# Thealexbarney/VGAudio

Hardware: NVIDIA H100
Metric: GC-ADPCM encode Msamples/sec (batch) (higher is better)
Workload: dtype int32

## Files before the change

include/vgaudio_b200.h:

```cpp
#ifndef VGAUDIO_B200_H
#define VGAUDIO_B200_H

#include <stdint.h>

#ifdef __cplusplus
extern "C" {
#endif

#define VGB_OK        0
#define VGB_E_ARG    -1
#define VGB_E_DATA   -2
#define VGB_E_STATE  -3
#define VGB_E_CUDA   -4
#define VGB_E_NCCL   -5
#define VGB_E_NOMEM  -6

#define VGB_ABI_VERSION 1

int32_t vgb_abi_version(void);
int32_t vgb_init(int32_t device, uint32_t flags);
int32_t vgb_shutdown(void);
int32_t vgb_init_devices(const int32_t *devices, int32_t n_devices, uint32_t flags);
int32_t vgb_device_count(void);

// ... 52 lines not shown
                               void *d_workspace, uint64_t workspace_bytes, void *cuda_stream);

int32_t vgb_gcadpcm_coefs_dev(const int16_t *d_pcm, const int64_t *pcm_offset, const int32_t *n_samples,
                              int32_t n_channels, int16_t *d_coefs_out,
                              void *d_workspace, uint64_t workspace_bytes, void *cuda_stream);

int32_t vgb_gcadpcm_decode_dev(const uint8_t *d_adpcm, const int64_t *adpcm_offset, const int16_t *d_coefs,
                               const vgb_gc_params *params , int32_t n_channels,
                               int16_t *d_pcm, const int64_t *pcm_offset,
                               void *d_workspace, uint64_t workspace_bytes, void *cuda_stream);
int32_t vgb_gcadpcm_decode_dev_status(const void *d_workspace, int32_t n_channels, void *cuda_stream);

typedef struct vgb_gc_tap_params {
    int32_t sample_count;
    int32_t samples_per_seek_table_entry;
    int32_t loop_start;
} vgb_gc_tap_params;

int32_t vgb_gcadpcm_seek_entry_count(int32_t sample_count, int32_t samples_per_entry);

int32_t vgb_gcadpcm_seek_context_batch(const uint8_t *const *adpcm, const int32_t *n_bytes, const int16_t *coefs,
                                       const vgb_gc_tap_params *params, int32_t n_channels,
                                       int16_t *const *seek_table_out, int16_t *loop_context_out);

typedef struct vgb_gc_align_params { int32_t multiple, loop_start, loop_end; } vgb_gc_align_params;
typedef struct vgb_gc_alignment { int32_t alignment_needed, loop_start_aligned, sample_count_aligned; } vgb_gc_alignment;

int32_t vgb_gcadpcm_alignment(const vgb_gc_align_params *p, vgb_gc_alignment *out);

int32_t vgb_gcadpcm_align_batch(const uint8_t *const *adpcm, const int32_t *n_bytes, const int16_t *coefs,
                                const vgb_gc_align_params *params, int32_t n_channels,
                                uint8_t *const *adpcm_aligned_out, int16_t *const *pcm_aligned_out);

int32_t vgb_interleave_dev(const void *d_in, int64_t in_channel_stride, int64_t in_item_stride, void *d_out, int64_t out_item_stride,
                           int32_t n_items, int32_t count, int64_t in_size, int32_t interleave_size, int64_t out_size, void *cuda_stream);
int32_t vgb_deinterleave_dev(const void *d_in, int64_t in_item_stride, void *d_out, int64_t out_channel_stride, int64_t out_item_stride,
                             int32_t n_items, int32_t count, int64_t in_size, int32_t interleave_size, int64_t out_size, void *cuda_stream);
int32_t vgb_interleave(const uint8_t *const *inputs, int32_t count, int32_t in_size, int32_t interleave_size, int32_t out_size,
                       uint8_t *output);
int32_t vgb_deinterleave(const uint8_t *input, int32_t length, int32_t interleave_size, int32_t count, int32_t out_size,
                         uint8_t *const *outputs);

int32_t vgb_set_kernel_timing(int32_t enabled);
int32_t vgb_last_kernel_ms(float *ms_out, int32_t n);

int32_t vgb_debug_last_timeline(float *ms_out, int32_t n);
int32_t vgb_debug_last_coefs_done(float *ms_out, int32_t n);

int32_t vgb_gcadpcm_debug_splice_stats(uint64_t *out, int32_t n);

int32_t vgb_gcadpcm_debug_records(const int16_t *pcm, int32_t n_samples, double *dir_out, uint8_t *accepted_out);
int32_t vgb_gcadpcm_debug_refine_trace(const int16_t *const *pcm, const int32_t *n_samples, int32_t n_channels, int32_t warps,
                                       double *cent_out, int32_t *hits_out, int16_t *coefs_out);


typedef struct vgb_adx_params {
    int32_t sample_rate;
    int32_t highpass_frequency;
    int32_t frame_size;
    int32_t version;
    int32_t history;
    int32_t padding;
    int32_t type;
    int32_t filter;
} vgb_adx_params;

int32_t vgb_adx_calculate_coefficients(int32_t highpass_frequency, int32_t sample_rate, int16_t *coefs_out);

int32_t vgb_adx_encoded_byte_count(int32_t pcm_length, int32_t padding, int32_t frame_size);

int32_t vgb_adx_encode_batch(const int16_t *const *pcm, const int32_t *n_samples, const vgb_adx_params *params,
                             int32_t n_channels, int16_t *history_out, uint8_t *const *adpcm_out,
                             vgb_progress_cb cb, void *user);

uint64_t vgb_adx_workspace_bytes(int64_t total_samples, int32_t n_channels);
int32_t vgb_adx_encode_dev(const int16_t *d_pcm, const int64_t *pcm_offset, const int32_t *n_samples, const vgb_adx_params *params,
                           int32_t n_channels, int16_t *d_history_out, uint8_t *d_adpcm, const int64_t *adpcm_offset,
                           void *d_workspace, uint64_t workspace_bytes, void *cuda_stream);

int32_t vgb_adx_decode_batch(const uint8_t *const *adpcm, const int32_t *n_bytes, const int32_t *sample_count,
                             const vgb_adx_params *params, int32_t n_channels, int16_t *const *pcm_out);

uint64_t vgb_adx_decode_workspace_bytes(const int32_t *sample_count, const vgb_adx_params *params, int32_t n_channels);
int32_t vgb_adx_decode_dev(const uint8_t *d_adpcm, const int64_t *adpcm_offset, const int32_t *n_bytes, const int32_t *sample_count,
                           const vgb_adx_params *params, int32_t n_channels, int16_t *d_pcm, const int64_t *pcm_offset,
                           void *d_workspace, uint64_t workspace_bytes, void *cuda_stream);
int32_t vgb_adx_decode_dev_status(const void *d_workspace, int32_t n_channels, void *cuda_stream);
int32_t vgb_adx_debug_decode_stats(uint64_t *out, int32_t n);


typedef struct vgb_hca_params {
    int32_t quality, bitrate, limit_bitrate;
    int32_t channel_count, sample_rate, sample_count;
    int32_t looping, loop_start, loop_end;
} vgb_hca_params;

typedef struct vgb_hca_info {
    int32_t channel_count, sample_rate, sample_count, frame_count, inserted_samples, appended_samples;
    int32_t header_size, frame_size, min_resolution, max_resolution, track_count, channel_config;
    int32_t total_band_count, base_band_count, stereo_band_count, hfr_band_count, bands_per_hfr_group, hfr_group_count;
    int32_t bitrate;
    int32_t looping, loop_start_frame, loop_end_frame, pre_loop_samples, post_loop_samples;
    int32_t use_ath_curve;
} vgb_hca_info;

int32_t vgb_hca_query(const vgb_hca_params *params, vgb_hca_info *info_out);
// ... 119 lines not shown
```

vgaudio_b200/_native.py:

```python
from __future__ import annotations

import ctypes as C
import os

_HERE = os.path.dirname(os.path.abspath(__file__))
LIB_PATH = os.path.join(_HERE, "libvgaudio_b200.so")

VGB_OK, VGB_E_ARG, VGB_E_DATA, VGB_E_STATE, VGB_E_CUDA, VGB_E_NCCL, VGB_E_NOMEM = 0, -1, -2, -3, -4, -5, -6


class VgbGcParams(C.Structure):

    _fields_ = [("sample_count", C.c_int32), ("history1", C.c_int16), ("history2", C.c_int16)]


class VgbAdxParams(C.Structure):

    _fields_ = [("sample_rate", C.c_int32), ("highpass_frequency", C.c_int32), ("frame_size", C.c_int32),
                ("version", C.c_int32), ("history", C.c_int32), ("padding", C.c_int32), ("type", C.c_int32),
                ("filter", C.c_int32)]


class VgbHcaParams(C.Structure):

# ... 125 lines not shown
    "vgb_gcadpcm_coefs_dev": (
        C.c_int32,
        [C.c_void_p, C.c_void_p, C.c_void_p, C.c_int32, C.c_void_p, C.c_void_p, C.c_uint64, C.c_void_p],
    ),
    "vgb_gcadpcm_decode_dev": (
        C.c_int32,
        [C.c_void_p, C.c_void_p, C.c_void_p, C.c_void_p, C.c_int32, C.c_void_p, C.c_void_p, C.c_void_p, C.c_uint64,
         C.c_void_p],
    ),
    "vgb_gcadpcm_decode_dev_status": (C.c_int32, [C.c_void_p, C.c_int32, C.c_void_p]),
    "vgb_adx_encoded_byte_count": (C.c_int32, [C.c_int32, C.c_int32, C.c_int32]),
    "vgb_adx_encode_batch": (C.c_int32, [C.c_void_p, C.c_void_p, C.c_void_p, C.c_int32, C.c_void_p, C.c_void_p,
                                         C.c_void_p, C.c_void_p]),
    "vgb_adx_calculate_coefficients": (C.c_int32, [C.c_int32, C.c_int32, C.c_void_p]),
    "vgb_adx_decode_batch": (C.c_int32, [C.c_void_p, C.c_void_p, C.c_void_p, C.c_void_p, C.c_int32, C.c_void_p]),
    "vgb_adx_decode_workspace_bytes": (C.c_uint64, [C.c_void_p, C.c_void_p, C.c_int32]),
    "vgb_adx_decode_dev": (C.c_int32, [C.c_void_p, C.c_void_p, C.c_void_p, C.c_void_p, C.c_void_p, C.c_int32, C.c_void_p, C.c_void_p,
                                       C.c_void_p, C.c_uint64, C.c_void_p]),
    "vgb_adx_decode_dev_status": (C.c_int32, [C.c_void_p, C.c_int32, C.c_void_p]),
    "vgb_adx_debug_decode_stats": (C.c_int32, [C.c_void_p, C.c_int32]),
    "vgb_adx_workspace_bytes": (C.c_uint64, [C.c_int64, C.c_int32]),
    "vgb_adx_encode_dev": (C.c_int32, [C.c_void_p, C.c_void_p, C.c_void_p, C.c_void_p, C.c_int32, C.c_void_p, C.c_void_p, C.c_void_p,
                                       C.c_void_p, C.c_uint64, C.c_void_p]),
    "vgb_hca_workspace_bytes": (C.c_uint64, [C.c_int32]),
    "vgb_hca_encode_dev": (C.c_int32, [C.c_void_p, C.c_void_p, C.c_void_p, C.c_void_p, C.c_int32, C.c_void_p, C.c_void_p, C.c_void_p,
                                       C.c_void_p, C.c_uint64, C.c_void_p]),
    "vgb_hca_encode_dev_status": (C.c_int32, [C.c_void_p, C.c_int32, C.c_void_p]),
    "vgb_mdct128_batch": (C.c_int32, [C.c_void_p, C.c_int32, C.c_int32, C.c_void_p]),
    "vgb_imdct128_batch": (C.c_int32, [C.c_void_p, C.c_int32, C.c_int32, C.c_void_p]),
    "vgb_hca_query": (C.c_int32, [C.c_void_p, C.c_void_p]),
    "vgb_hca_encode_batch": (C.c_int32, [C.c_void_p, C.c_void_p, C.c_int32, C.c_void_p, C.c_void_p, C.c_void_p, C.c_void_p]),
    "vgb_hca_decode_batch": (C.c_int32, [C.c_void_p, C.c_void_p, C.c_int32, C.c_void_p]),
    "vgb_hca_decode_workspace_bytes": (C.c_uint64, [C.c_void_p, C.c_int32]),
    "vgb_hca_decode_dev": (C.c_int32, [C.c_void_p, C.c_void_p, C.c_void_p, C.c_int32, C.c_void_p, C.c_void_p, C.c_void_p, C.c_void_p,
                                       C.c_uint64, C.c_void_p]),
    "vgb_hca_decode_dev_status": (C.c_int32, [C.c_void_p, C.c_int32, C.c_void_p]),
    "vgb_gcadpcm_seek_entry_count": (C.c_int32, [C.c_int32, C.c_int32]),
    "vgb_gcadpcm_seek_context_batch": (C.c_int32, [C.c_void_p, C.c_void_p, C.c_void_p, C.c_void_p, C.c_int32, C.c_void_p, C.c_void_p]),
    "vgb_gcadpcm_alignment": (C.c_int32, [C.c_void_p, C.c_void_p]),
    "vgb_gcadpcm_align_batch": (C.c_int32, [C.c_void_p, C.c_void_p, C.c_void_p, C.c_void_p, C.c_int32, C.c_void_p, C.c_void_p]),
    "vgb_interleave_dev": (C.c_int32, [C.c_void_p, C.c_int64, C.c_int64, C.c_void_p, C.c_int64, C.c_int32, C.c_int32, C.c_int64,
                                       C.c_int32, C.c_int64, C.c_void_p]),
    "vgb_deinterleave_dev": (C.c_int32, [C.c_void_p, C.c_int64, C.c_void_p, C.c_int64, C.c_int64, C.c_int32, C.c_int32, C.c_int64,
                                         C.c_int32, C.c_int64, C.c_void_p]),
    "vgb_interleave": (C.c_int32, [C.c_void_p, C.c_int32, C.c_int32, C.c_int32, C.c_int32, C.c_void_p]),
    "vgb_deinterleave": (C.c_int32, [C.c_void_p, C.c_int32, C.c_int32, C.c_int32, C.c_int32, C.c_void_p]),
    "vgb_set_kernel_timing": (C.c_int32, [C.c_int32]),
    "vgb_last_kernel_ms": (C.c_int32, [C.c_void_p, C.c_int32]),
    "vgb_debug_last_timeline": (C.c_int32, [C.c_void_p, C.c_int32]),
    "vgb_debug_last_coefs_done": (C.c_int32, [C.c_void_p, C.c_int32]),
    "vgb_gcadpcm_debug_records": (C.c_int32, [C.c_void_p, C.c_int32, C.c_void_p, C.c_void_p]),
    "vgb_gcadpcm_debug_refine_trace": (C.c_int32, [C.c_void_p, C.c_void_p, C.c_int32, C.c_int32, C.c_void_p, C.c_void_p,
                                                   C.c_void_p]),
    "vgb_gcadpcm_debug_splice_stats": (C.c_int32, [C.c_void_p, C.c_int32]),
    "vgb_wave_parse": (C.c_int32, [C.c_void_p, C.c_int64, C.c_void_p]),
    "vgb_wave_read_batch": (C.c_int32, [C.c_void_p, C.c_void_p, C.c_void_p, C.c_int32, C.c_void_p]),
    "vgb_dsp_file_size": (C.c_int64, [C.c_void_p]),
    "vgb_dsp_write_batch": (C.c_int32, [C.c_void_p, C.c_int32, C.c_void_p, C.c_void_p, C.c_void_p, C.c_void_p, C.c_void_p, C.c_void_p]),
    "vgb_dsp_parse": (C.c_int32, [C.c_void_p, C.c_int64, C.c_void_p]),
    "vgb_dsp_read_batch": (C.c_int32, [C.c_void_p, C.c_void_p, C.c_void_p, C.c_int32, C.c_void_p]),
    "vgb_adx_key_from_code": (C.c_int32, [C.c_uint64, C.c_void_p]),
    "vgb_adx_key_from_string": (C.c_int32, [C.c_char_p, C.c_void_p]),
    "vgb_adx_file_size": (C.c_int64, [C.c_void_p]),
    "vgb_adx_write_batch": (C.c_int32, [C.c_void_p, C.c_int32, C.c_void_p, C.c_void_p, C.c_void_p, C.c_void_p, C.c_void_p]),
    "vgb_adx_crypt_batch": (C.c_int32, [C.c_void_p, C.c_int32, C.c_int32, C.c_void_p, C.c_int32, C.c_int32]),
    "vgb_adx_parse": (C.c_int32, [C.c_void_p, C.c_int64, C.c_void_p]),
    "vgb_hca_parse": (C.c_int32, [C.c_void_p, C.c_int64, C.c_void_p, C.c_void_p]),
    "vgb_hca_key_tables": (C.c_int32, [C.c_int32, C.c_uint64, C.c_void_p, C.c_void_p]),
    "vgb_hca_crypt_batch": (C.c_int32, [C.c_void_p, C.c_void_p, C.c_int32, C.c_int32, C.c_int32, C.c_uint64, C.c_int32]),
    "vgb_hca_write_batch": (C.c_int32, [C.c_void_p, C.c_int32, C.c_void_p, C.c_int32, C.c_uint64, C.c_void_p, C.c_void_p, C.c_void_p]),
    "vgb_convert_debug_stage_ms": (C.c_int32, [C.c_void_p, C.c_int32]),
    "vgb_convert_dsp_to_wave_batch": (C.c_int32, [C.c_void_p, C.c_void_p, C.c_int32, C.c_void_p, C.c_void_p, C.c_void_p]),
    "vgb_convert_hca_to_wave_batch": (C.c_int32, [C.c_void_p, C.c_void_p, C.c_int32, C.c_void_p, C.c_void_p, C.c_void_p, C.c_void_p]),
    "vgb_convert_adx_to_wave_batch": (C.c_int32, [C.c_void_p, C.c_void_p, C.c_int32, C.c_void_p, C.c_void_p, C.c_void_p, C.c_void_p]),
    "vgb_convert_wave_batch": (C.c_int32, [C.c_void_p, C.c_void_p, C.c_int32, C.c_void_p, C.c_void_p, C.c_void_p, C.c_void_p,
                                           C.c_void_p, C.c_void_p]),
    "vgb_transcode_batch": (C.c_int32, [C.c_void_p, C.c_void_p, C.c_void_p, C.c_int32, C.c_void_p, C.c_void_p, C.c_void_p,
                                        C.c_void_p, C.c_void_p, C.c_void_p, C.c_void_p, C.c_void_p]),
}


class VgbError(RuntimeError):

    def __init__(self, code: int, message: str):
        super().__init__(f"vgaudio_b200 error {code}: {message}")
        self.code = code


def _load() -> C.CDLL:
    if not os.path.exists(LIB_PATH):
        raise ImportError(
            f"{LIB_PATH} is missing: build it with `python -c 'import __graft_entry__ as g; g.build()'` "
            "(nvcc, sm_90a).  vgaudio_b200 has no CPU fallback."
        )
    lib = C.CDLL(LIB_PATH)
    for name, (res, args) in SIGNATURES.items():
        fn = getattr(lib, name)
        fn.restype = res
        fn.argtypes = args
    return lib


lib = _load()


def check(status: int) -> None:
# ... 3 lines not shown
```

vgaudio_b200/csrc/abi_gcadpcm.cu:

```cuda
#include <climits>

#include "abi.cuh"

using namespace vgb;

namespace {

struct GcLayout {
    int32_t n_channels = 0;
    std::vector<int64_t> pcm_off, adpcm_off, rec_off;
    std::vector<int32_t> n_samples, enc_count;
    std::vector<int16_t> hist;
    int64_t pcm_total = 0;
    int64_t adpcm_total = 0;
    int64_t rec_total = 0;
    int32_t max_frames = 0;
    int64_t total_frames = 0;
};

struct GcWorkspace {
    size_t off_pcm_off, off_adpcm_off, off_rec_off, off_n_samples, off_enc_count, off_hist, off_records, off_mask;
    size_t off_trace, off_used_start, off_stats;
    size_t off_status;
    size_t table_bytes;
// ... 923 lines not shown
    CUDA_TRY(cudaGetLastError());
    std::vector<uint32_t> mask((size_t)frames / 32 + 1);
    CUDA_TRY(cudaMemcpyAsync(dir_out, b + w.off_records, (size_t)frames * 16, cudaMemcpyDeviceToHost, st));
    CUDA_TRY(cudaMemcpyAsync(mask.data(), b + w.off_mask, mask.size() * 4, cudaMemcpyDeviceToHost, st));
    CUDA_TRY(cudaStreamSynchronize(st));
    for (int f = 0; f < frames; f++) accepted_out[f] = (mask[f >> 5] >> (f & 31)) & 1u;
    return VGB_OK;
}

int32_t vgb_gcadpcm_debug_refine_trace(const int16_t *const *pcm, const int32_t *n_samples, int32_t n_channels, int32_t warps,
                                       double *cent_out, int32_t *hits_out, int16_t *coefs_out)
{
    if (n_channels < 0 || (warps != 4 && warps != 8) || !cent_out || !hits_out || !coefs_out)
        return fail(VGB_E_ARG, "bad arguments");
    if (n_channels == 0) return VGB_OK;
    if (!pcm) return fail(VGB_E_ARG, "pcm is NULL");
    GcLayout lay;
    VGB_TRY(layout_common(lay, n_samples, nullptr, n_channels, false));
    for (int c = 0; c < n_channels; c++)
        if (!pcm[c] && lay.n_samples[c] > 0) return fail(VGB_E_ARG, "pcm[%d] is NULL", c);
    layout_pack_offsets(lay);
    std::vector<int64_t> pcm_b(n_channels), pcm_len(n_channels);
    for (int c = 0; c < n_channels; c++) {
        pcm_b[c] = lay.pcm_off[c] * 2;
        pcm_len[c] = (int64_t)lay.n_samples[c] * 2;
    }
    std::lock_guard<std::mutex> lock(g_ctx.mu);
    VGB_TRY(ensure_ready_locked());
    cudaStream_t st = g_ctx.stream;
    const GcWorkspace w = carve(lay.rec_total, n_channels);
    const size_t n = (size_t)n_channels, cent_bytes = n * 7 * 8 * 2 * 8, hits_bytes = n * 7 * 8 * 4;
    VGB_TRY(g_ctx.pcm.reserve((size_t)lay.pcm_total * 2));
    VGB_TRY(g_ctx.ws.reserve(w.total));
    VGB_TRY(g_ctx.coefs.reserve(n * 32));
    VGB_TRY(g_ctx.misc.reserve(align_up(cent_bytes, 256) + hits_bytes));
    double *d_cent = reinterpret_cast<double *>(g_ctx.misc.p);
    int32_t *d_hits = reinterpret_cast<int32_t *>(g_ctx.misc.c() + align_up(cent_bytes, 256));
    VGB_TRY(copy_units(cudaMemcpyHostToDevice, g_ctx.pcm.c(), pcm_b.data(), pcm, pcm_len.data(), 0, n_channels, st));
    VGB_TRY(upload_tables(lay, w, g_ctx.ws.p, st));
    GcChannelTable tab = table_view(g_ctx.ws.p, w, n_channels);
    double2 *records = reinterpret_cast<double2 *>(g_ctx.ws.c() + w.off_records);
    uint32_t *mask = reinterpret_cast<uint32_t *>(g_ctx.ws.c() + w.off_mask);
    launch_gc_coef_frames(static_cast<const int16_t *>(g_ctx.pcm.p), tab, records, mask, lay.max_frames, 0, INT_MAX, st);
    launch_gc_coef_refine_tap(tab, records, mask, static_cast<int16_t *>(g_ctx.coefs.p), warps, d_cent, d_hits, st);
    g_ctx.launches += (lay.max_frames > 0 ? 1 : 0) + 1;
    CUDA_TRY(cudaGetLastError());
    CUDA_TRY(cudaMemcpyAsync(cent_out, d_cent, cent_bytes, cudaMemcpyDeviceToHost, st));
    CUDA_TRY(cudaMemcpyAsync(hits_out, d_hits, hits_bytes, cudaMemcpyDeviceToHost, st));
    CUDA_TRY(cudaMemcpyAsync(coefs_out, g_ctx.coefs.p, n * 32, cudaMemcpyDeviceToHost, st));
    CUDA_TRY(cudaStreamSynchronize(st));
    return VGB_OK;
}

}
```

vgaudio_b200/csrc/gc_coefs.cu:

```cuda
#include "common.cuh"
#include <cstdlib>

#include "kernels.h"

namespace vgb {

constexpr int kP1Threads = 256;
constexpr int kP1TileSamples = kP1Threads * kGcFrameSamples;


__device__ __forceinline__ bool gc_frame_direct(const int32_t (&x)[16], double &d1, double &d2)
{
    long long s0 = 0, s1 = 0, s2 = 0;
#pragma unroll
    for (int t = 0; t < 14; t++) {
        long long a = x[t + 2];
        s0 += a * x[t + 2];
        s1 += a * x[t + 1];
        s2 += a * x[t];
    }
    double v0 = 0.0 - (double)s0;
    double v1 = 0.0 - (double)s1;
    double v2 = 0.0 - (double)s2;
    if (!(fabs(v0) > 10.0)) return false;
// ... 128 lines not shown
struct Centroid {
    double e0, e1, e2;
};

__device__ __forceinline__ void gc_finish(double k1, double k2, double &o1, double &o2)
{
    if (k1 >= 1.0) k1 = 0.9999999999; else if (k1 <= -1.0) k1 = -0.9999999999;
    if (k2 >= 1.0) k2 = 0.9999999999; else if (k2 <= -1.0) k2 = -0.9999999999;
    o1 = (k2 * k1) + k1;
    o2 = k2;
}

__device__ __forceinline__ void gc_centroid_from_mean(double s0, double s1, double s2, double &o1, double &o2)
{
    double err = s0;
    double acc = 0.0;
    double t1 = (err > 0.0) ? (-(acc + s1) / err) : 0.0;
    double k1 = t1;
    err *= 1.0 - (t1 * t1);
    acc = 0.0;
    acc += t1 * s1;
    double t2 = (err > 0.0) ? (-(acc + s2) / err) : 0.0;
    double k2 = t2;
    gc_finish(k1, k2, o1, o2);
}

__device__ __forceinline__ int16_t gc_quantise_coef(double v)
{
    double d = -v * 2048.0;
    if (d > 0.0) return d > 32767.0 ? (int16_t)32767 : (int16_t)__double2int_rn(d);
    if (d < -32768.0) return (int16_t)-32768;
    if (d != d) return 0;
    return (int16_t)__double2int_rn(d);
}


struct __align__(16) RefineSlot {
    double2 q[8 * 33];
    int32_t count[8];
};
__host__ __device__ constexpr int refine_row(int nb) { return nb >= 8 ? 33 : (nb == 4 ? 66 : (nb == 2 ? 132 : 264)); }
__host__ __device__ constexpr int refine_step(int nb) { return nb >= 4 ? 4 : (nb == 2 ? 8 : 16); }

template <int W>
struct RefineShared {
    RefineSlot slot[2][W - 1];
    double cent[8][3];
    double econst[8][3];
};

template <int W>
__device__ __forceinline__ void refine_chunk_barrier() { asm volatile("bar.sync 1, %0;" ::"n"(W * 32) : "memory"); }

struct RefineSum { double acc; int hits; };
template <int NB, int W>
__device__ __forceinline__ RefineSum gc_refine_consume(int lane, int n_blocks, int n_chunks, RefineShared<W> &sh)
{
    constexpr int P = W - 1;
    constexpr int STEP = refine_step(NB), ROW = refine_row(NB);
    const int my_bucket = (lane >> 1) & 7, my_comp = lane & 1;
    double a = 0.0;
    int h = 0;
    refine_chunk_barrier<W>();
    for (int c = 1; c <= n_chunks; c++) {
        const int first = (c - 1) * P;
        for (int j = 0; j < P && first + j < n_blocks; j++) {
            const RefineSlot &slot = sh.slot[(c - 1) & 1][j];
            const int n_mine = (lane < 16 && my_bucket < NB) ? slot.count[my_bucket] : 0;
            const double *col = reinterpret_cast<const double *>(slot.q + (my_bucket < NB ? my_bucket : 0) * ROW) + my_comp;
            const int n_pad = (n_mine + STEP - 1) / STEP * STEP;
            for (int j0 = 0; j0 < n_pad; j0 += STEP) {
                double v[STEP];
#pragma unroll
                for (int i = 0; i < STEP; i++) v[i] = col[2 * (j0 + i)];
#pragma unroll
                for (int i = 0; i < STEP; i++) a += v[i];
            }
            h += n_mine;
        }
        refine_chunk_barrier<W>();
    }
    return RefineSum{a, h};
}

template <int COUNT, int W>
__device__ __forceinline__ void gc_refine_pass(int warp, int lane, int n_frames, int n_blocks, const double2 *__restrict__ rec,
                                               const uint32_t *__restrict__ mask, RefineShared<W> &sh, double &acc, int &hits)
{
    constexpr int NB = COUNT > 0 ? COUNT : 1;
    constexpr int P = W - 1;
    constexpr int STEP = refine_step(NB), ROW = refine_row(NB);
    const uint32_t lanes_below = (1u << lane) - 1u;
    const int p = warp - 1;
    const int n_chunks = (n_blocks + P - 1) / P;

    auto fetch = [&](int b, double2 &r, uint32_t &okbits) {
        r = make_double2(0.0, 0.0);
        okbits = 0;
        if (warp > 0 && b < n_blocks) {
            okbits = mask[b];
            const int f = b * 32 + lane;
            if (f < n_frames) r = rec[f];
        }
    };
    auto stage = [&](int b, double2 r, uint32_t okbits, RefineSlot &slot) {
        const bool ok = ((okbits >> lane) & 1u) && (b * 32 + lane < n_frames);
        int pick = 0;
        if (COUNT > 1) {
            const double ta = 2.0 * r.x, tb = 2.0 * r.y;
            double d[NB];
            int idx[NB];
#pragma unroll
            for (int i = 0; i < NB; i++) {
                const double di = sh.econst[i][0] + (ta * sh.econst[i][1]) + (tb * sh.econst[i][2]);
                d[i] = di < 1.0e30 ? di : __longlong_as_double(0x7FF0000000000000ll);
                idx[i] = i;
            }
#pragma unroll
            for (int step = 1; step < NB; step *= 2) {
#pragma unroll
                for (int i = 0; i + step < NB; i += 2 * step) {
                    const bool right = d[i + step] < d[i];
                    d[i] = right ? d[i + step] : d[i];
                    idx[i] = right ? idx[i + step] : idx[i];
                }
            }
            pick = d[0] < 1.0e30 ? idx[0] : 0;
        }
        if (lane < NB) slot.count[lane] = 0;
        const uint32_t mine = __match_any_sync(0xFFFFFFFFu, ok ? pick : NB);
        __syncwarp();
        if (ok) {
            const int rank = __popc(mine & lanes_below);
            if (rank == 0) slot.count[pick] = __popc(mine);
            slot.q[pick * ROW + rank] = r;
        }
        __syncwarp();
        {
            const int bucket = lane / STEP, i = lane % STEP;
            if (bucket < NB) {
                const int c = slot.count[bucket];
                if (i < ((STEP - (c % STEP)) % STEP)) slot.q[bucket * ROW + c + i] = make_double2(-0.0, -0.0);
            }
        }
    };
    acc = 0.0;
    hits = 0;
    constexpr int kDepth = 4;
    double2 ring_r[kDepth];
    uint32_t ring_ok[kDepth];
#pragma unroll
    for (int k = 0; k < kDepth; k++) fetch(p + k * P, ring_r[k], ring_ok[k]);

    if (warp == 0) {
        const RefineSum sum = gc_refine_consume<NB, W>(lane, n_blocks, n_chunks, sh);
        acc = sum.acc;
        hits = sum.hits;
        return;
    }
    for (int c0 = 0; c0 <= n_chunks; c0 += kDepth) {
#pragma unroll
        for (int k = 0; k < kDepth; k++) {
            const int c = c0 + k;
            if (c > n_chunks) break;
            const int b = c * P + p;
            if (b < n_blocks) stage(b, ring_r[k], ring_ok[k], sh.slot[c & 1][p]);
            fetch(b + kDepth * P, ring_r[k], ring_ok[k]);
            refine_chunk_barrier<W>();
        }
    }
}

template <int W, bool kTap>
__device__ __forceinline__ void gc_coef_refine(GcChannelTable tab, const double2 *__restrict__ records,
                                               const uint32_t *__restrict__ accept_mask, int16_t *__restrict__ coefs_out,
                                               double *__restrict__ tap_cent, int32_t *__restrict__ tap_hits)
{
    extern __shared__ __align__(16) unsigned char refine_smem[];
    RefineShared<W> &sh = *reinterpret_cast<RefineShared<W> *>(refine_smem);
    constexpr int kRefineProducers = W - 1;

    const int warp = threadIdx.x >> 5, lane = threadIdx.x & 31;
    const int ch = blockIdx.x;
    if (ch >= tab.n_channels) return;

    double (*best)[3] = sh.cent;
    const int n_frames = div_round_up(tab.n_samples[ch], kGcFrameSamples);
    const int n_blocks = (n_frames + 31) >> 5;
    const double2 *rec = records + tab.rec_off[ch];
    const uint32_t *mask = accept_mask + (tab.rec_off[ch] >> 5);

    if (threadIdx.x < 8) { best[threadIdx.x][0] = 1.0; best[threadIdx.x][1] = 0.0; best[threadIdx.x][2] = 0.0; }
    if (threadIdx.x < 2 * kRefineProducers * 8) sh.slot[threadIdx.x / (kRefineProducers * 8)][(threadIdx.x / 8) % kRefineProducers].count[threadIdx.x & 7] = 0;
    __syncthreads();

    int count = 1;
    for (int pass = 0; pass < 7; pass++) {
        if (pass == 1 || pass == 3 || pass == 5) {
            if (warp == 0 && lane < count) {
                best[count + lane][0] = (0.01 * 0.0) + best[lane][0];
                best[count + lane][1] = (0.01 * -1.0) + best[lane][1];
                best[count + lane][2] = (0.01 * 0.0) + best[lane][2];
            }
            count *= 2;
            __syncthreads();
        }
        if (warp == 0 && lane < count) {
            const double a0 = best[lane][0], a1 = best[lane][1], a2 = best[lane][2];
            sh.econst[lane][0] = (a0 * a0) + (a1 * a1) + (a2 * a2);
            sh.econst[lane][1] = (a0 * a1) + (a1 * a2);
            sh.econst[lane][2] = a0 * a2;
        }
        __syncthreads();
        double acc;
        int hits;
        if (pass == 0) gc_refine_pass<0, W>(warp, lane, n_frames, n_blocks, rec, mask, sh, acc, hits);
        else if (count == 2) gc_refine_pass<2, W>(warp, lane, n_frames, n_blocks, rec, mask, sh, acc, hits);
        else if (count == 4) gc_refine_pass<4, W>(warp, lane, n_frames, n_blocks, rec, mask, sh, acc, hits);
        else gc_refine_pass<8, W>(warp, lane, n_frames, n_blocks, rec, mask, sh, acc, hits);

        if (warp == 0) {
            double mean;
            if (pass == 0) mean = acc / (double)hits;
            else mean = hits > 0 ? acc / (double)hits : acc;
            const double m1 = __shfl_sync(0xFFFFFFFFu, mean, (lane & 7) * 2);
            const double m2 = __shfl_sync(0xFFFFFFFFu, mean, (lane & 7) * 2 + 1);
            const int h = __shfl_sync(0xFFFFFFFFu, hits, (lane & 7) * 2);
            if (lane < count) {
                const double m0 = (pass == 0) ? 1.0 : (h > 0 ? 1.0 : 0.0);
                double o1, o2;
                gc_centroid_from_mean(m0, m1, m2, o1, o2);
                best[lane][0] = 1.0;
                best[lane][1] = o1;
                best[lane][2] = o2;
            }
            if (kTap && lane < 8) {
                const int64_t at = ((int64_t)ch * 7 + pass) * 8 + lane;
                tap_cent[2 * at] = best[lane][1];
                tap_cent[2 * at + 1] = best[lane][2];
                tap_hits[at] = h;
            }
        }
        __syncthreads();
    }

    if (threadIdx.x < 16) coefs_out[(int64_t)ch * 16 + threadIdx.x] = gc_quantise_coef(best[threadIdx.x >> 1][1 + (threadIdx.x & 1)]);
}

template <int W>
__global__ void __launch_bounds__(W * 32, W == 4 ? 8 : 3)
gc_coef_refine_kernel(GcChannelTable tab, const double2 *__restrict__ records, const uint32_t *__restrict__ accept_mask,
                      int16_t *__restrict__ coefs_out)
{
    gc_coef_refine<W, false>(tab, records, accept_mask, coefs_out, nullptr, nullptr);
}

template <int W>
__global__ void __launch_bounds__(W * 32, W == 4 ? 8 : 3)
gc_coef_refine_tap_kernel(GcChannelTable tab, const double2 *__restrict__ records, const uint32_t *__restrict__ accept_mask,
                          int16_t *__restrict__ coefs_out, double *__restrict__ tap_cent, int32_t *__restrict__ tap_hits)
{
    gc_coef_refine<W, true>(tab, records, accept_mask, coefs_out, tap_cent, tap_hits);
}

void launch_gc_coef_frames(const int16_t *pcm, const GcChannelTable &tab, double2 *records, uint32_t *mask,
                           int max_frames, int frame_begin, int frame_end, cudaStream_t stream)
{
    if (tab.n_channels <= 0 || max_frames <= 0) return;
    int hi = frame_end < max_frames ? frame_end : max_frames;
    if (hi <= frame_begin) return;
    int tiles = (hi - frame_begin + kP1Threads - 1) / kP1Threads;
    if (tiles > 65535) tiles = 65535;
    dim3 grid((unsigned)tab.n_channels, (unsigned)tiles);
    gc_coef_frames_kernel<<<grid, kP1Threads, 0, stream>>>(pcm, tab, records, mask, frame_begin, frame_end);
}

void launch_gc_coef_refine(const GcChannelTable &tab, const double2 *records, const uint32_t *mask,
                           int16_t *coefs_out, cudaStream_t stream)
{
    if (tab.n_channels <= 0) return;
    static int wide_limit = -1;
    if (wide_limit < 0) {
        wide_limit = 0;
        if (const char *env = std::getenv("VGB_REFINE_WIDE_LIMIT")) wide_limit = std::atoi(env);
    }
    if (tab.n_channels <= wide_limit) {
        raise_dynamic_smem(gc_coef_refine_kernel<8>, sizeof(RefineShared<8>));
        gc_coef_refine_kernel<8><<<tab.n_channels, 8 * 32, sizeof(RefineShared<8>), stream>>>(tab, records, mask, coefs_out);
    } else {
        raise_dynamic_smem(gc_coef_refine_kernel<4>, sizeof(RefineShared<4>));
        gc_coef_refine_kernel<4><<<tab.n_channels, 4 * 32, sizeof(RefineShared<4>), stream>>>(tab, records, mask, coefs_out);
    }
}

void launch_gc_coef_refine_tap(const GcChannelTable &tab, const double2 *records, const uint32_t *mask, int16_t *coefs_out,
                               int warps, double *tap_cent, int32_t *tap_hits, cudaStream_t stream)
{
    if (tab.n_channels <= 0) return;
    if (warps == 8) {
        raise_dynamic_smem(gc_coef_refine_tap_kernel<8>, sizeof(RefineShared<8>));
        gc_coef_refine_tap_kernel<8><<<tab.n_channels, 8 * 32, sizeof(RefineShared<8>), stream>>>(tab, records, mask, coefs_out,
                                                                                                  tap_cent, tap_hits);
    } else {
        raise_dynamic_smem(gc_coef_refine_tap_kernel<4>, sizeof(RefineShared<4>));
        gc_coef_refine_tap_kernel<4><<<tab.n_channels, 4 * 32, sizeof(RefineShared<4>), stream>>>(tab, records, mask, coefs_out,
                                                                                                  tap_cent, tap_hits);
    }
}

}
```

vgaudio_b200/csrc/kernels.h:

```cpp
#pragma once

#include <cuda_runtime.h>
#include <stdint.h>

#include "common.cuh"

namespace vgb {

cudaError_t raise_dynamic_smem(const void *kernel, size_t bytes);
template <class Kernel>
cudaError_t raise_dynamic_smem(Kernel *kernel, size_t bytes) { return raise_dynamic_smem(reinterpret_cast<const void *>(kernel), bytes); }

void launch_gc_coef_frames(const int16_t *pcm, const GcChannelTable &tab, double2 *records, uint32_t *mask,
                           int max_frames, int frame_begin, int frame_end, cudaStream_t stream);
void launch_gc_coef_refine(const GcChannelTable &tab, const double2 *records, const uint32_t *mask,
                           int16_t *coefs_out, cudaStream_t stream);
void launch_gc_coef_refine_tap(const GcChannelTable &tab, const double2 *records, const uint32_t *mask, int16_t *coefs_out,
                               int warps, double *tap_cent, int32_t *tap_hits, cudaStream_t stream);

int gc_encode_pick_segments(int n_channels, int max_frames, int *min_seg_out = nullptr);
void launch_gc_encode(const int16_t *pcm, const GcChannelTable &tab, const int16_t *coefs, uint8_t *adpcm,
                      int max_frames, int frame_begin, int frame_end, GcSegArgs seg, cudaStream_t stream);
void launch_gc_encode_frames(int16_t *pcm_in_out, const int32_t *sample_count, const int16_t *coefs, int n_frames,
                             uint8_t *adpcm_out, cudaStream_t stream);

void launch_gc_decode(const uint8_t *adpcm, const GcChannelTable &tab, const int16_t *coefs, int16_t *pcm,
                      int max_frames, int frame_begin, int frame_end, cudaStream_t stream);

void launch_gc_taps(const uint8_t *adpcm, const GcChannelTable &tab, const int16_t *coefs, const GcTapChannel *taps,
                    int16_t *tap_slab, int max_frames, cudaStream_t stream);

void launch_gc_align_tail(const int16_t *pcm, const GcAlignChannel *chans, int n_channels, int16_t *tail, int16_t *hist_enc,
                          int16_t *hist_dec, cudaStream_t stream);

int adx_encode_pick_segments(int n_channels, int max_whole_frames, int *min_seg_out = nullptr);
void launch_adx_encode(const int16_t *pcm, const AdxChannel *tab, int n_channels, uint8_t *adpcm, int16_t *history_out,
                       AdxSegArgs seg, cudaStream_t stream);
void launch_adx_decode(const uint8_t *adpcm, const AdxChannel *tab, int n_channels, int16_t *pcm, int32_t *status,
                       cudaStream_t stream);
int adx_decode_pick_segments(int n_channels, int max_body_frames, int *min_seg_out);
void launch_adx_decode_seg(const uint8_t *adpcm, const AdxDecChannel *tab, int n_channels, int16_t *pcm, AdxDecSegArgs seg,
                           cudaStream_t stream);

size_t hca_encode_smem_bytes(const HcaConfig &cfg);
cudaError_t launch_hca_encode(const int16_t *pcm, const HcaStream *streams, int n_streams, int max_frames,
                              const HcaConfig &cfg, const HcaTables &tables, uint8_t *frames_out, int32_t *status_out,
                              cudaStream_t stream);

size_t hca_decode_smem_bytes(const HcaConfig &cfg);
size_t hca_decode_parsed_bytes(const HcaConfig &cfg, int64_t total_frames);
cudaError_t launch_hca_decode(const uint8_t *frames, const HcaStream *streams, int n_streams, int max_frames,
                              int64_t total_frames, const HcaConfig &cfg, const HcaTables &tables, uint8_t *parsed_scratch,
                              double *edge_scratch, int16_t *pcm, int32_t *status_out,
                              cudaStream_t stream);

cudaError_t launch_hca_mdct128(const double *in, double *out, int n_sequences, int n_blocks, bool inverse, const HcaTables &tables,
                               cudaStream_t stream);

cudaError_t launch_interleave(const void *in, int64_t in_channel_stride, int64_t in_item_stride, void *out, int64_t out_item_stride,
                              int n_items, int count, int64_t in_size, int64_t interleave, int64_t out_size, cudaStream_t stream);
cudaError_t launch_deinterleave(const void *in, int64_t in_item_stride, void *out, int64_t out_channel_stride, int64_t out_item_stride,
                                int n_items, int count, int64_t in_size, int64_t interleave, int64_t out_size, cudaStream_t stream);

}
```

Baseline: 31670.

## Restructure refine consumer into flattened prefetched groups and add timing probe kernel

Rewrites the refine consumer warp to flatten all producer slots in a chunk into one group sequence of up to eight doubles, software-prefetching the next group while summing the current one. Producers now issue the next fetch before classifying the current block, and the prefetch ring depth drops from four to two. It also adds a clock-instrumented probe kernel and a debug entry point that time the refine stages. The aim is to cut consumer load latency and per-slot loop overhead, with the risk that the shallower fetch ring exposes global load latency.

```diff
diff --git a/include/vgaudio_b200.h b/include/vgaudio_b200.h
--- a/include/vgaudio_b200.h
+++ b/include/vgaudio_b200.h
@@ -128,6 +128,10 @@
 int32_t vgb_gcadpcm_debug_records(const int16_t *pcm, int32_t n_samples, double *dir_out, uint8_t *accepted_out);
 int32_t vgb_gcadpcm_debug_refine_trace(const int16_t *const *pcm, const int32_t *n_samples, int32_t n_channels, int32_t warps,
                                        double *cent_out, int32_t *hits_out, int16_t *coefs_out);
+int32_t vgb_gcadpcm_debug_refine_probe(const int16_t *d_pcm, const int64_t *pcm_offset, const int32_t *n_samples,
+                                       int32_t n_channels, int32_t warps, int32_t reps, void *d_workspace,
+                                       uint64_t workspace_bytes, int64_t *sums_out, uint32_t *hist_out, float *ms_out,
+                                       int32_t *ctas_per_sm_out);
 
 
 typedef struct vgb_adx_params {
diff --git a/vgaudio_b200/_native.py b/vgaudio_b200/_native.py
--- a/vgaudio_b200/_native.py
+++ b/vgaudio_b200/_native.py
@@ -201,6 +201,8 @@
     "vgb_gcadpcm_debug_records": (C.c_int32, [C.c_void_p, C.c_int32, C.c_void_p, C.c_void_p]),
     "vgb_gcadpcm_debug_refine_trace": (C.c_int32, [C.c_void_p, C.c_void_p, C.c_int32, C.c_int32, C.c_void_p, C.c_void_p,
                                                    C.c_void_p]),
+    "vgb_gcadpcm_debug_refine_probe": (C.c_int32, [C.c_void_p, C.c_void_p, C.c_void_p, C.c_int32, C.c_int32, C.c_int32, C.c_void_p,
+                                                   C.c_uint64, C.c_void_p, C.c_void_p, C.c_void_p, C.c_void_p]),
     "vgb_gcadpcm_debug_splice_stats": (C.c_int32, [C.c_void_p, C.c_int32]),
     "vgb_wave_parse": (C.c_int32, [C.c_void_p, C.c_int64, C.c_void_p]),
     "vgb_wave_read_batch": (C.c_int32, [C.c_void_p, C.c_void_p, C.c_void_p, C.c_int32, C.c_void_p]),
diff --git a/vgaudio_b200/csrc/abi_gcadpcm.cu b/vgaudio_b200/csrc/abi_gcadpcm.cu
--- a/vgaudio_b200/csrc/abi_gcadpcm.cu
+++ b/vgaudio_b200/csrc/abi_gcadpcm.cu
@@ -999,4 +999,58 @@
     return VGB_OK;
 }
 
-}
+int32_t vgb_gcadpcm_debug_refine_probe(const int16_t *d_pcm, const int64_t *pcm_offset, const int32_t *n_samples,
+                                       int32_t n_channels, int32_t warps, int32_t reps, void *d_workspace,
+                                       uint64_t workspace_bytes, int64_t *sums_out, uint32_t *hist_out, float *ms_out,
+                                       int32_t *ctas_per_sm_out)
+{
+    if (n_channels <= 0 || (warps != 4 && warps != 8) || reps <= 0 || !sums_out || !hist_out || !ms_out || !ctas_per_sm_out)
+        return fail(VGB_E_ARG, "bad arguments");
+    GcLayout lay;
+    VGB_TRY(dev_layout(lay, pcm_offset, nullptr, n_samples, nullptr, n_channels, false, false));
+    if (!d_pcm || !d_workspace) return fail(VGB_E_ARG, "NULL device pointer");
+    VGB_TRY(check_aligned(d_pcm, 16, "d_pcm"));
+    VGB_TRY(check_aligned(d_workspace, 16, "d_workspace"));
+    const GcWorkspace w = carve(lay.rec_total, n_channels);
+    if (w.total > workspace_bytes)
+        return fail(VGB_E_ARG, "workspace too small: need %zu bytes, got %llu", w.total, (unsigned long long)workspace_bytes);
+    int sums_words = 0, hist_words = 0;
+    refine_probe_sizes(warps, &sums_words, &hist_words);
+    const size_t n = (size_t)n_channels, sums_bytes = n * sums_words * 8, hist_bytes = (size_t)hist_words * 4;
+    std::lock_guard<std::mutex> lock(g_ctx.mu);
+    VGB_TRY(ensure_ready_locked());
+    cudaStream_t st = g_ctx.stream;
+    VGB_TRY(g_ctx.coefs.reserve(n * 32));
+    VGB_TRY(g_ctx.misc.reserve(align_up(sums_bytes, 256) + hist_bytes));
+    long long *d_sums = reinterpret_cast<long long *>(g_ctx.misc.p);
+    uint32_t *d_hist = reinterpret_cast<uint32_t *>(g_ctx.misc.c() + align_up(sums_bytes, 256));
+    int16_t *d_coefs = static_cast<int16_t *>(g_ctx.coefs.p);
+    VGB_TRY(upload_tables(lay, w, d_workspace, st));
+    GcChannelTable tab = table_view(d_workspace, w, n_channels);
+    double2 *records = reinterpret_cast<double2 *>(static_cast<char *>(d_workspace) + w.off_records);
+    uint32_t *mask = reinterpret_cast<uint32_t *>(static_cast<char *>(d_workspace) + w.off_mask);
+    launch_gc_coef_frames(d_pcm, tab, records, mask, lay.max_frames, 0, INT_MAX, st);
+    CUDA_TRY(cudaMemsetAsync(g_ctx.misc.p, 0, align_up(sums_bytes, 256) + hist_bytes, st));
+    cudaEvent_t ev[4];
+    for (auto &e : ev) CUDA_TRY(cudaEventCreate(&e));
+    struct Events { cudaEvent_t *e; ~Events() { for (int i = 0; i < 4; i++) cudaEventDestroy(e[i]); } } free_events{ev};
+    launch_gc_coef_refine_width(tab, records, mask, d_coefs, warps, st);
+    CUDA_TRY(cudaEventRecord(ev[0], st));
+    for (int r = 0; r < reps; r++) launch_gc_coef_refine_width(tab, records, mask, d_coefs, warps, st);
+    CUDA_TRY(cudaEventRecord(ev[1], st));
+    CUDA_TRY(cudaEventRecord(ev[2], st));
+    launch_gc_coef_refine_probe(tab, records, mask, d_coefs, warps, d_sums, d_hist, st);
+    CUDA_TRY(cudaEventRecord(ev[3], st));
+    g_ctx.launches += (lay.max_frames > 0 ? 1 : 0) + reps + 2;
+    CUDA_TRY(cudaGetLastError());
+    CUDA_TRY(cudaMemcpyAsync(sums_out, d_sums, sums_bytes, cudaMemcpyDeviceToHost, st));
+    CUDA_TRY(cudaMemcpyAsync(hist_out, d_hist, hist_bytes, cudaMemcpyDeviceToHost, st));
+    CUDA_TRY(cudaStreamSynchronize(st));
+    CUDA_TRY(cudaEventElapsedTime(&ms_out[0], ev[0], ev[1]));
+    CUDA_TRY(cudaEventElapsedTime(&ms_out[1], ev[2], ev[3]));
+    ms_out[0] /= (float)reps;
+    CUDA_TRY(refine_probe_occupancy(warps, &ctas_per_sm_out[0], &ctas_per_sm_out[1]));
+    return VGB_OK;
+}
+
+}
diff --git a/vgaudio_b200/csrc/gc_coefs.cu b/vgaudio_b200/csrc/gc_coefs.cu
--- a/vgaudio_b200/csrc/gc_coefs.cu
+++ b/vgaudio_b200/csrc/gc_coefs.cu
@@ -204,40 +204,97 @@
 template <int W>
 __device__ __forceinline__ void refine_chunk_barrier() { asm volatile("bar.sync 1, %0;" ::"n"(W * 32) : "memory"); }
 
+enum class RefineMode { kPlain, kTap, kProbe };
+
+constexpr int kProbeBins = 64, kProbeBinShift = 6;
+enum RefineProbeQty { kQConsumerAdd, kQConsumerBarrier, kQProducerFetch, kQProducerClassify, kQProducerBarrier, kProbeQty };
+constexpr int kProbeWords = 5;
+struct RefineProbe {
+    long long fetch, work, wait;
+    int chunks;
+    uint32_t sink;
+    uint32_t *hist;
+    __device__ __forceinline__ void bin(int q, uint32_t cycles, int lane) const
+    {
+        if (lane == 0) atomicAdd(&hist[q * kProbeBins + min(cycles >> kProbeBinShift, (uint32_t)kProbeBins - 1)], 1u);
+    }
+};
+template <RefineMode M>
+__device__ __forceinline__ uint32_t probe_clock() { return M == RefineMode::kProbe ? (uint32_t)clock() : 0u; }
+
 struct RefineSum { double acc; int hits; };
-template <int NB, int W>
-__device__ __forceinline__ RefineSum gc_refine_consume(int lane, int n_blocks, int n_chunks, RefineShared<W> &sh)
+template <int NB, int W, RefineMode M>
+__device__ __forceinline__ RefineSum gc_refine_consume(int lane, int n_blocks, int n_chunks, RefineShared<W> &sh, RefineProbe &pr)
 {
     constexpr int P = W - 1;
     constexpr int STEP = refine_step(NB), ROW = refine_row(NB);
+    constexpr int CG = STEP < 8 ? STEP : 8;
     const int my_bucket = (lane >> 1) & 7, my_comp = lane & 1;
     double a = 0.0;
     int h = 0;
+    uint32_t t0 = probe_clock<M>();
     refine_chunk_barrier<W>();
+    if constexpr (M == RefineMode::kProbe) {
+        const uint32_t t = probe_clock<M>();
+        pr.wait += t - t0;
+        t0 = t;
+    }
     for (int c = 1; c <= n_chunks; c++) {
-        const int first = (c - 1) * P;
-        for (int j = 0; j < P && first + j < n_blocks; j++) {
-            const RefineSlot &slot = sh.slot[(c - 1) & 1][j];
-            const int n_mine = (lane < 16 && my_bucket < NB) ? slot.count[my_bucket] : 0;
-            const double *col = reinterpret_cast<const double *>(slot.q + (my_bucket < NB ? my_bucket : 0) * ROW) + my_comp;
-            const int n_pad = (n_mine + STEP - 1) / STEP * STEP;
-            for (int j0 = 0; j0 < n_pad; j0 += STEP) {
-                double v[STEP];
-#pragma unroll
-                for (int i = 0; i < STEP; i++) v[i] = col[2 * (j0 + i)];
-#pragma unroll
-                for (int i = 0; i < STEP; i++) a += v[i];
-            }
-            h += n_mine;
-        }
-        refine_chunk_barrier<W>();
+        const RefineSlot *slot = sh.slot[(c - 1) & 1];
+        const int in_chunk = min(P, n_blocks - (c - 1) * P);
+        int g_lo[P], g_hi[P], n_groups = 0;
+#pragma unroll
+        for (int j = 0; j < P; j++) {
+            const int n = (j < in_chunk && lane < 16 && my_bucket < NB) ? slot[j].count[my_bucket] : 0;
+            h += n;
+            g_lo[j] = n_groups;
+            n_groups += (n + STEP - 1) / STEP * (STEP / CG);
+            g_hi[j] = n_groups;
+        }
+        const double *col = reinterpret_cast<const double *>(slot[0].q + (my_bucket < NB ? my_bucket : 0) * ROW) + my_comp;
+        auto group = [&](int g) {
+            const double *at = col;
+#pragma unroll
+            for (int j = 0; j < P; j++)
+                if (g >= g_lo[j] && g < g_hi[j]) at = col + j * (int)(sizeof(RefineSlot) / sizeof(double)) + 2 * CG * (g - g_lo[j]);
+            return at;
+        };
+        double v[CG];
+        const double *at = group(0);
+#pragma unroll
+        for (int i = 0; i < CG; i++) v[i] = at[2 * i];
+        for (int g = 0; g < n_groups; g++) {
+            double w[CG];
+            at = group(g + 1);
+#pragma unroll
+            for (int i = 0; i < CG; i++) w[i] = at[2 * i];
+#pragma unroll
+            for (int i = 0; i < CG; i++) a += v[i];
+#pragma unroll
+            for (int i = 0; i < CG; i++) v[i] = w[i];
+        }
+        if constexpr (M == RefineMode::kProbe) {
+            pr.sink ^= (uint32_t)__double_as_longlong(a);
+            const uint32_t t1 = probe_clock<M>();
+            refine_chunk_barrier<W>();
+            const uint32_t t2 = probe_clock<M>();
+            pr.work += t1 - t0;
+            pr.wait += t2 - t1;
+            pr.chunks++;
+            pr.bin(kQConsumerAdd, t1 - t0, lane);
+            pr.bin(kQConsumerBarrier, t2 - t1, lane);
+            t0 = t2;
+        } else {
+            refine_chunk_barrier<W>();
+        }
     }
     return RefineSum{a, h};
 }
 
-template <int COUNT, int W>
+template <int COUNT, int W, RefineMode M>
 __device__ __forceinline__ void gc_refine_pass(int warp, int lane, int n_frames, int n_blocks, const double2 *__restrict__ rec,
-                                               const uint32_t *__restrict__ mask, RefineShared<W> &sh, double &acc, int &hits)
+                                               const uint32_t *__restrict__ mask, RefineShared<W> &sh, double &acc, int &hits,
+                                               RefineProbe &pr)
 {
     constexpr int NB = COUNT > 0 ? COUNT : 1;
     constexpr int P = W - 1;
@@ -255,7 +312,8 @@
             if (f < n_frames) r = rec[f];
         }
     };
-    auto stage = [&](int b, double2 r, uint32_t okbits, RefineSlot &slot) {
+    struct Picked { bool ok; int pick; uint32_t mine; };
+    auto classify = [&](int b, double2 r, uint32_t okbits, RefineSlot &slot) {
         const bool ok = ((okbits >> lane) & 1u) && (b * 32 + lane < n_frames);
         int pick = 0;
         if (COUNT > 1) {
@@ -281,6 +339,12 @@
         }
         if (lane < NB) slot.count[lane] = 0;
         const uint32_t mine = __match_any_sync(0xFFFFFFFFu, ok ? pick : NB);
+        return Picked{ok, pick, mine};
+    };
+    auto enqueue = [&](Picked k, double2 r, RefineSlot &slot) {
+        const bool ok = k.ok;
+        const int pick = k.pick;
+        const uint32_t mine = k.mine;
         __syncwarp();
         if (ok) {
             const int rank = __popc(mine & lanes_below);
@@ -298,39 +362,62 @@
     };
     acc = 0.0;
     hits = 0;
-    constexpr int kDepth = 4;
+    constexpr int kDepth = 2;
     double2 ring_r[kDepth];
     uint32_t ring_ok[kDepth];
 #pragma unroll
     for (int k = 0; k < kDepth; k++) fetch(p + k * P, ring_r[k], ring_ok[k]);
 
     if (warp == 0) {
-        const RefineSum sum = gc_refine_consume<NB, W>(lane, n_blocks, n_chunks, sh);
+        const RefineSum sum = gc_refine_consume<NB, W, M>(lane, n_blocks, n_chunks, sh, pr);
         acc = sum.acc;
         hits = sum.hits;
         return;
     }
+    uint32_t t0 = probe_clock<M>();
     for (int c0 = 0; c0 <= n_chunks; c0 += kDepth) {
 #pragma unroll
         for (int k = 0; k < kDepth; k++) {
             const int c = c0 + k;
             if (c > n_chunks) break;
             const int b = c * P + p;
-            if (b < n_blocks) stage(b, ring_r[k], ring_ok[k], sh.slot[c & 1][p]);
+            uint32_t t1 = 0, t2 = 0;
+            if constexpr (M == RefineMode::kProbe) {
+                pr.sink ^= ring_ok[k] ^ (uint32_t)__double_as_longlong(ring_r[k].x) ^ (uint32_t)__double_as_longlong(ring_r[k].y);
+                t1 = probe_clock<M>();
+            }
+            const double2 r = ring_r[k];
+            const uint32_t okbits = ring_ok[k];
             fetch(b + kDepth * P, ring_r[k], ring_ok[k]);
+            if (b < n_blocks) enqueue(classify(b, r, okbits, sh.slot[c & 1][p]), r, sh.slot[c & 1][p]);
+            if constexpr (M == RefineMode::kProbe) t2 = probe_clock<M>();
             refine_chunk_barrier<W>();
-        }
-    }
-}
-
-template <int W, bool kTap>
+            if constexpr (M == RefineMode::kProbe) {
+                const uint32_t t3 = probe_clock<M>();
+                pr.fetch += t1 - t0;
+                pr.work += t2 - t1;
+                pr.wait += t3 - t2;
+                pr.chunks++;
+                pr.bin(kQProducerFetch, t1 - t0, lane);
+                pr.bin(kQProducerClassify, t2 - t1, lane);
+                pr.bin(kQProducerBarrier, t3 - t2, lane);
+                t0 = t3;
+            }
+        }
+    }
+}
+
+template <int W, RefineMode M>
 __device__ __forceinline__ void gc_coef_refine(GcChannelTable tab, const double2 *__restrict__ records,
                                                const uint32_t *__restrict__ accept_mask, int16_t *__restrict__ coefs_out,
-                                               double *__restrict__ tap_cent, int32_t *__restrict__ tap_hits)
+                                               double *__restrict__ tap_cent, int32_t *__restrict__ tap_hits,
+                                               long long *__restrict__ probe_sums, uint32_t *__restrict__ probe_hist)
 {
     extern __shared__ __align__(16) unsigned char refine_smem[];
     RefineShared<W> &sh = *reinterpret_cast<RefineShared<W> *>(refine_smem);
     constexpr int kRefineProducers = W - 1;
+    constexpr bool kTap = M == RefineMode::kTap;
+    RefineProbe pr{0, 0, 0, 0, 0, reinterpret_cast<uint32_t *>(refine_smem + sizeof(RefineShared<W>))};
 
     const int warp = threadIdx.x >> 5, lane = threadIdx.x & 31;
     const int ch = blockIdx.x;
@@ -344,6 +431,8 @@
 
     if (threadIdx.x < 8) { best[threadIdx.x][0] = 1.0; best[threadIdx.x][1] = 0.0; best[threadIdx.x][2] = 0.0; }
     if (threadIdx.x < 2 * kRefineProducers * 8) sh.slot[threadIdx.x / (kRefineProducers * 8)][(threadIdx.x / 8) % kRefineProducers].count[threadIdx.x & 7] = 0;
+    if constexpr (M == RefineMode::kProbe)
+        for (int i = threadIdx.x; i < kProbeQty * kProbeBins; i += W * 32) pr.hist[i] = 0;
     __syncthreads();
 
     int count = 1;
@@ -366,10 +455,10 @@
         __syncthreads();
         double acc;
         int hits;
-        if (pass == 0) gc_refine_pass<0, W>(warp, lane, n_frames, n_blocks, rec, mask, sh, acc, hits);
-        else if (count == 2) gc_refine_pass<2, W>(warp, lane, n_frames, n_blocks, rec, mask, sh, acc, hits);
-        else if (count == 4) gc_refine_pass<4, W>(warp, lane, n_frames, n_blocks, rec, mask, sh, acc, hits);
-        else gc_refine_pass<8, W>(warp, lane, n_frames, n_blocks, rec, mask, sh, acc, hits);
+        if (pass == 0) gc_refine_pass<0, W, M>(warp, lane, n_frames, n_blocks, rec, mask, sh, acc, hits, pr);
+        else if (count == 2) gc_refine_pass<2, W, M>(warp, lane, n_frames, n_blocks, rec, mask, sh, acc, hits, pr);
+        else if (count == 4) gc_refine_pass<4, W, M>(warp, lane, n_frames, n_blocks, rec, mask, sh, acc, hits, pr);
+        else gc_refine_pass<8, W, M>(warp, lane, n_frames, n_blocks, rec, mask, sh, acc, hits, pr);
 
         if (warp == 0) {
             double mean;
@@ -394,6 +483,23 @@
             }
         }
         __syncthreads();
+        if constexpr (M == RefineMode::kProbe) {
+            if (lane == 0) {
+                long long *o = probe_sums + (((int64_t)ch * 7 + pass) * W + warp) * kProbeWords;
+                o[0] = pr.fetch;
+                o[1] = pr.work;
+                o[2] = pr.wait;
+                o[3] = pr.chunks;
+                o[4] = pr.sink;
+            }
+            pr.fetch = pr.work = pr.wait = 0;
+            pr.chunks = 0;
+            for (int i = threadIdx.x; i < kProbeQty * kProbeBins; i += W * 32) {
+                const uint32_t v = pr.hist[i];
+                if (v) atomicAdd(&probe_hist[pass * kProbeQty * kProbeBins + i], v);
+                pr.hist[i] = 0;
+            }
+        }
     }
 
     if (threadIdx.x < 16) coefs_out[(int64_t)ch * 16 + threadIdx.x] = gc_quantise_coef(best[threadIdx.x >> 1][1 + (threadIdx.x & 1)]);
@@ -404,7 +510,7 @@
 gc_coef_refine_kernel(GcChannelTable tab, const double2 *__restrict__ records, const uint32_t *__restrict__ accept_mask,
                       int16_t *__restrict__ coefs_out)
 {
-    gc_coef_refine<W, false>(tab, records, accept_mask, coefs_out, nullptr, nullptr);
+    gc_coef_refine<W, RefineMode::kPlain>(tab, records, accept_mask, coefs_out, nullptr, nullptr, nullptr, nullptr);
 }
 
 template <int W>
@@ -412,7 +518,15 @@
 gc_coef_refine_tap_kernel(GcChannelTable tab, const double2 *__restrict__ records, const uint32_t *__restrict__ accept_mask,
                           int16_t *__restrict__ coefs_out, double *__restrict__ tap_cent, int32_t *__restrict__ tap_hits)
 {
-    gc_coef_refine<W, true>(tab, records, accept_mask, coefs_out, tap_cent, tap_hits);
+    gc_coef_refine<W, RefineMode::kTap>(tab, records, accept_mask, coefs_out, tap_cent, tap_hits, nullptr, nullptr);
+}
+
+template <int W>
+__global__ void __launch_bounds__(W * 32, W == 4 ? 8 : 3)
+gc_coef_refine_probe_kernel(GcChannelTable tab, const double2 *__restrict__ records, const uint32_t *__restrict__ accept_mask,
+                            int16_t *__restrict__ coefs_out, long long *__restrict__ probe_sums, uint32_t *__restrict__ probe_hist)
+{
+    gc_coef_refine<W, RefineMode::kProbe>(tab, records, accept_mask, coefs_out, nullptr, nullptr, probe_sums, probe_hist);
 }
 
 void launch_gc_coef_frames(const int16_t *pcm, const GcChannelTable &tab, double2 *records, uint32_t *mask,
@@ -436,13 +550,7 @@
         wide_limit = 0;
         if (const char *env = std::getenv("VGB_REFINE_WIDE_LIMIT")) wide_limit = std::atoi(env);
     }
-    if (tab.n_channels <= wide_limit) {
-        raise_dynamic_smem(gc_coef_refine_kernel<8>, sizeof(RefineShared<8>));
-        gc_coef_refine_kernel<8><<<tab.n_channels, 8 * 32, sizeof(RefineShared<8>), stream>>>(tab, records, mask, coefs_out);
-    } else {
-        raise_dynamic_smem(gc_coef_refine_kernel<4>, sizeof(RefineShared<4>));
-        gc_coef_refine_kernel<4><<<tab.n_channels, 4 * 32, sizeof(RefineShared<4>), stream>>>(tab, records, mask, coefs_out);
-    }
+    launch_gc_coef_refine_width(tab, records, mask, coefs_out, tab.n_channels <= wide_limit ? 8 : 4, stream);
 }
 
 void launch_gc_coef_refine_tap(const GcChannelTable &tab, const double2 *records, const uint32_t *mask, int16_t *coefs_out,
@@ -460,4 +568,60 @@
     }
 }
 
-}
+void refine_probe_sizes(int warps, int *sums_words, int *hist_words)
+{
+    *sums_words = 7 * warps * kProbeWords;
+    *hist_words = 7 * kProbeQty * kProbeBins;
+}
+
+template <int W, typename K>
+static cudaError_t refine_occupancy(K kernel, size_t smem, int *out)
+{
+    raise_dynamic_smem(kernel, smem);
+    return cudaOccupancyMaxActiveBlocksPerMultiprocessor(out, kernel, W * 32, smem);
+}
+
+cudaError_t refine_probe_occupancy(int warps, int *plain_ctas, int *probe_ctas)
+{
+    const size_t hist = kProbeQty * kProbeBins * sizeof(uint32_t);
+    cudaError_t e;
+    if (warps == 8) {
+        e = refine_occupancy<8>(gc_coef_refine_kernel<8>, sizeof(RefineShared<8>), plain_ctas);
+        if (e == cudaSuccess) e = refine_occupancy<8>(gc_coef_refine_probe_kernel<8>, sizeof(RefineShared<8>) + hist, probe_ctas);
+    } else {
+        e = refine_occupancy<4>(gc_coef_refine_kernel<4>, sizeof(RefineShared<4>), plain_ctas);
+        if (e == cudaSuccess) e = refine_occupancy<4>(gc_coef_refine_probe_kernel<4>, sizeof(RefineShared<4>) + hist, probe_ctas);
+    }
+    return e;
+}
+
+void launch_gc_coef_refine_width(const GcChannelTable &tab, const double2 *records, const uint32_t *mask, int16_t *coefs_out,
+                                 int warps, cudaStream_t stream)
+{
+    if (tab.n_channels <= 0) return;
+    if (warps == 8) {
+        raise_dynamic_smem(gc_coef_refine_kernel<8>, sizeof(RefineShared<8>));
+        gc_coef_refine_kernel<8><<<tab.n_channels, 8 * 32, sizeof(RefineShared<8>), stream>>>(tab, records, mask, coefs_out);
+    } else {
+        raise_dynamic_smem(gc_coef_refine_kernel<4>, sizeof(RefineShared<4>));
+        gc_coef_refine_kernel<4><<<tab.n_channels, 4 * 32, sizeof(RefineShared<4>), stream>>>(tab, records, mask, coefs_out);
+    }
+}
+
+void launch_gc_coef_refine_probe(const GcChannelTable &tab, const double2 *records, const uint32_t *mask, int16_t *coefs_out,
+                                 int warps, long long *probe_sums, uint32_t *probe_hist, cudaStream_t stream)
+{
+    if (tab.n_channels <= 0) return;
+    const size_t hist = kProbeQty * kProbeBins * sizeof(uint32_t);
+    if (warps == 8) {
+        raise_dynamic_smem(gc_coef_refine_probe_kernel<8>, sizeof(RefineShared<8>) + hist);
+        gc_coef_refine_probe_kernel<8><<<tab.n_channels, 8 * 32, sizeof(RefineShared<8>) + hist, stream>>>(
+            tab, records, mask, coefs_out, probe_sums, probe_hist);
+    } else {
+        raise_dynamic_smem(gc_coef_refine_probe_kernel<4>, sizeof(RefineShared<4>) + hist);
+        gc_coef_refine_probe_kernel<4><<<tab.n_channels, 4 * 32, sizeof(RefineShared<4>) + hist, stream>>>(
+            tab, records, mask, coefs_out, probe_sums, probe_hist);
+    }
+}
+
+}
diff --git a/vgaudio_b200/csrc/kernels.h b/vgaudio_b200/csrc/kernels.h
--- a/vgaudio_b200/csrc/kernels.h
+++ b/vgaudio_b200/csrc/kernels.h
@@ -17,6 +17,12 @@
                            int16_t *coefs_out, cudaStream_t stream);
 void launch_gc_coef_refine_tap(const GcChannelTable &tab, const double2 *records, const uint32_t *mask, int16_t *coefs_out,
                                int warps, double *tap_cent, int32_t *tap_hits, cudaStream_t stream);
+void launch_gc_coef_refine_width(const GcChannelTable &tab, const double2 *records, const uint32_t *mask, int16_t *coefs_out,
+                                 int warps, cudaStream_t stream);
+void launch_gc_coef_refine_probe(const GcChannelTable &tab, const double2 *records, const uint32_t *mask, int16_t *coefs_out,
+                                 int warps, long long *probe_sums, uint32_t *probe_hist, cudaStream_t stream);
+void refine_probe_sizes(int warps, int *sums_words, int *hist_words);
+cudaError_t refine_probe_occupancy(int warps, int *plain_ctas, int *probe_ctas);
 
 int gc_encode_pick_segments(int n_channels, int max_frames, int *min_seg_out = nullptr);
 void launch_gc_encode(const int16_t *pcm, const GcChannelTable &tab, const int16_t *coefs, uint8_t *adpcm,
```

Result: faster. 32730, median of 6 (+3.4%).
